# Stability-AI/stable-audio-tools

Measured on AMD Instinct MI355X. Metric: train-step samples/sec (47s@44.1kHz), higher is better.
Workload: dtype f32(bf16x3)

## Files before the change

### include/sat_amd.h

```cpp
#ifndef SAT_AMD_H
#define SAT_AMD_H

#ifdef __cplusplus
extern "C" {
#endif

int sat_abi_version(void);
int sat_is_simulator(void);
const char* sat_last_error(void);


int sat_conv1d(const float* x, const float* w_packed, const float* bias, const float* alpha, const float* beta,
               const float* res, float* y, const float* x2, const float* alpha2, const float* beta2,
               float* part_da, float* part_db, int B, int Cin, int Cout, int Tin, int Tout, int K, int stride,
               int dil, int pad, int tanh_out, void* stream);
int sat_conv1d_partial_rows(int B, int Tout);

int sat_conv1d_bf16x3(const float* x, const short* w_hi, const short* w_lo, const float* bias, const float* snake_a,
                      const float* snake_ib, const float* res, float* y, const float* x2, const float* alpha2,
                      const float* beta2, float* part_da, float* part_db, int B, int Cin, int Cout, int Tin, int Tout,
                      int K, int stride, int dil, int pad, int tanh_out, void* stream);
int sat_conv1d_bf16x3_emit(const float* x, const short* w_hi, const short* w_lo, const float* bias, const float* snake_a,
                      const float* snake_ib, const float* res, float* y, const float* x2, const float* alpha2,
                      const float* beta2, float* part_da, float* part_db, int B, int Cin, int Cout, int Tin, int Tout,
// ... 28 lines not shown
                  void* em_lo, int B, int Cin, int Cout, int frames, int W, int kh, int kw, int dil_t, float slope, const float* lk_src,
                  float lk_slope, void* stream);
int sat_disc_wgrad_nsplit(int B, int M, int Cin, int kh, int frames, int W);
int sat_disc_wgrad(const float* dy, const float* x, float* partial, int B, int M, int Cin, int frames, int W, int kh, int kw, int dil_t,
                   void* stream);

int sat_conv1d_k7_plane_rows(int Tin, int Tout, int pad);
int sat_conv1d_k7_planes(const float* x, const float* snake_a, const float* snake_ib, short* xp_hi, short* xp_lo, int B, int Cin, int Tin,
                         int rows, void* stream);
long long sat_pack_weights_k7q_size(int D0, int D1, int K, int mode);
int sat_pack_weights_k7q(const float* w, short* hi, short* lo, int D0, int D1, int K, int mode, void* stream);
int sat_conv1d_bf16x3_planesq(const short* xp_hi, const short* xp_lo, int rows, const short* w_hi, const short* w_lo, const float* bias,
                             const float* res, float* y, const float* x2, const float* alpha2, const float* beta2, float* part_da,
                             float* part_db, int B, int Cin, int Cout, int Tin, int Tout, int K, int dil, int pad, int tanh_out,
                             int flags, void* stream);
int sat_convtr1d_bf16x3_partial_rows(int B, int Tout, int stride, int pad);
int sat_pack_weights_bf16x3(const float* w, short* hi, short* lo, int D0, int D1, int K, int stride, int mode, void* stream);
long long sat_pack_weights_bf16x3_size(int D0, int D1, int K, int stride, int mode);
int sat_snake_consts(const float* alpha, const float* beta, float* a, float* ib, int C, void* stream);

int sat_convtr1d(const float* x, const float* w_packed, const float* bias, const float* alpha, const float* beta,
                 const float* res, float* y, const float* x2, const float* alpha2, const float* beta2,
                 float* part_da, float* part_db, int B, int Cin, int Cout, int Tin, int Tout, int K, int stride,
                 int pad, int tanh_out, void* stream);
int sat_convtr1d_partial_rows(int B, int Tout, int stride, int pad);

int sat_conv_wgrad(const float* lo, const float* hi, const float* alpha, const float* beta, int snake_on,
                   float* partial, long long so_m, long long so_n, long long so_k, int B, int M, int N, int Tlo,
                   int Thi, int K, int stride, int dil, int pad, void* stream);
int sat_conv_wgrad_nsplit(int B, int M, int N, int Tlo, int K, int stride, int dil);
// ... 162 lines not shown
```

### stable_audio_tools_amd/_lib.py

```python
import ctypes
import os

_P = ctypes.c_void_p
_I = ctypes.c_int
_L = ctypes.c_longlong
_F = ctypes.c_float

SIGNATURES = {
    "sat_abi_version": (_I, []),
    "sat_is_simulator": (_I, []),
    "sat_last_error": (ctypes.c_char_p, []),
    "sat_conv1d": (_I, [_P] * 12 + [_I] * 10 + [_P]),
    "sat_conv1d_partial_rows": (_I, [_I, _I]),
    "sat_conv1d_bf16x3": (_I, [_P] * 13 + [_I] * 10 + [_P]),
    "sat_conv1d_bf16x3_emit": (_I, [_P] * 13 + [_I] * 10 + [_P] * 4 + [_I, _P]),
    "sat_convtr1d_bf16x3": (_I, [_P] * 13 + [_I] * 9 + [_P]),
    "sat_conv1d_bf16x3_partial_rows": (_I, [_I] * 4),
    "sat_rows_pack": (_I, [_P, _P] + [_I] * 10 + [_P]),
    "sat_rows_pack_bwd": (_I, [_P, _P] + [_I] * 10 + [_P]),
    "sat_rows_unpack": (_I, [_P, _P] + [_I] * 6 + [_F, _P]),
    "sat_rows_unpack_bwd": (_I, [_P, _P, _P] + [_I] * 6 + [_F, _P]),
    "sat_disc_geom": (_I, [_I, _I, _P, _P, _P, _P]),
    "sat_disc_planes": (_I, [_P] * 7 + [_I] * 5 + [_F, _P]),
    "sat_disc_l1_blocks": (_I, []),
    "sat_disc_l1_sum": (_I, [_P, _P, _P, _P, _L, _P]),
    "sat_disc_pack_size": (_L, [_I] * 5),
    "sat_disc_pack_weights": (_I, [_P] * 2 + [_I] * 5 + [_P]),
    "sat_disc_conv": (_I, [_P] * 7 + [_I] * 8 + [_F, _P, _F, _P]),
    "sat_disc_wgrad_nsplit": (_I, [_I] * 6),
    "sat_disc_wgrad": (_I, [_P] * 3 + [_I] * 8 + [_P]),
    "sat_conv1d_k7_plane_rows": (_I, [_I] * 3),
    "sat_conv1d_k7_planes": (_I, [_P] * 5 + [_I] * 4 + [_P]),
    "sat_conv1d_bf16x3_planesq": (_I, [_P, _P, _I] + [_P] * 10 + [_I] * 10 + [_P]),
    "sat_pack_weights_k7q": (_I, [_P, _P, _P, _I, _I, _I, _I, _P]),
    "sat_residual_unit_fwd": (_I, [_P, _P, _I] + [_P] * 11 + [_I] * 6 + [_P] * 4 + [_I, _P]),
    "sat_pack_weights_k7q_size": (_L, [_I, _I, _I, _I]),
    "sat_convtr1d_bf16x3_partial_rows": (_I, [_I] * 4),
    "sat_pack_weights_bf16x3": (_I, [_P, _P, _P, _I, _I, _I, _I, _I, _P]),
    "sat_pack_weights_bf16x3_size": (_L, [_I, _I, _I, _I, _I]),
    "sat_snake_consts": (_I, [_P, _P, _P, _P, _I, _P]),
    "sat_conv_wgrad7_bf16x3": (_I, [_P] * 5 + [_L] * 3 + [_I] * 6 + [_P, _P]),
    "sat_conv_wgrad7_bf16x3_nsplit": (_I, [_I] * 4),
    "sat_conv_wgrad7_bf16x3_fuses_rowsum": (_I, [_I] * 4),
    "sat_conv_wgrad_bf16x3": (_I, [_P] * 4 + [_I, _P] + [_L] * 3 + [_I] * 8 + [_P, _P]),
    "sat_conv_wgrad_bf16x3_nsplit": (_I, [_I] * 6),
    "sat_convtr1d": (_I, [_P] * 12 + [_I] * 9 + [_P]),
    "sat_convtr1d_partial_rows": (_I, [_I, _I, _I, _I]),
    "sat_conv_wgrad": (_I, [_P, _P, _P, _P, _I, _P, _L, _L, _L] + [_I] * 9 + [_P]),
    "sat_conv_wgrad_nsplit": (_I, [_I] * 7),
    "sat_reduce_splits": (_I, [_P, _P, _L, _I, _F, _I, _P]),
    "sat_ru_k1_bwd_nsplit": (_I, [_I] * 3),
# ... 101 lines not shown
```

### stable_audio_tools_amd/csrc/conv1d_bf16x3.hip

```cpp
#include "conv_common.h"
#include <type_traits>

#define SAT_K7P_LEAD_ROWS 32
#define SAT_BF_AROWS1 192
#define SAT_BF_AROWSN 136

struct SatConvBfLaunch {
    SatConvParams p;
    const short* w_hi;
    const short* w_lo;
    int cout_pad;
    int cin_v, cout_v;
    int sin_log2;
    int sout_log2;
    int in_shift, out_shift;
    int nq;
    const short* xp_hi = nullptr;
    const short* xp_lo = nullptr;
    int xp_rows = 0, xp_c8 = 0;
    int wq = 0;
    int stagger = 0;
    int persist = 0;
    int dma_in_mfma = 0;
    short* em_hi = nullptr;
    short* em_lo = nullptr;
    const float* em_a = nullptr;
    const float* em_ib = nullptr;
    int em_rows = 0, em_c8 = 0;
    const short* ru_w1_hi = nullptr;
    const short* ru_w1_lo = nullptr;
    const float* ru_bias2 = nullptr;
    const float* ru_a2 = nullptr;
    const float* ru_ib2 = nullptr;
    float* ru_h = nullptr;
};

SAT_DEVICE void sat_split2(float x, short* hi, short* lo) {
    const short h = sat_f32_to_bf16(x);
// ... 672 lines not shown
    if (!em_hi) { sat_set_error("sat_conv1d_bf16x3_emit: planes missing"); return 1; }
    return sat_conv1d_bf16x3_impl("sat_conv1d_bf16x3_emit", x, w_hi, w_lo, bias, snake_a, snake_ib, res, y, x2, alpha2, beta2, part_da, part_db,
                                  B, Cin, Cout, Tin, Tout, K, stride, dil, pad, tanh_out, (short*)em_hi, (short*)em_lo, em_a, em_ib, em_rows, stream);
}

extern "C" int sat_conv1d_k7_plane_rows(int Tin, int Tout, int pad) {
    if (Tin <= 0 || Tout <= 0 || pad < 0 || pad > SAT_K7P_LEAD) return -1;
    const int need = sat_cdiv(Tout, SAT_K7_T) * SAT_K7_T - pad + SAT_K7_AROWS;
    const int body = need > Tin ? need : Tin;
    return SAT_K7P_LEAD + sat_cdiv(body, 64) * 64;
}
extern "C" int sat_conv1d_k7_planes(const float* x, const float* snake_a, const float* snake_ib, short* xp_hi, short* xp_lo, int B,
                                    int Cin, int Tin, int rows, void* stream) {
    if (B <= 0 || Cin <= 0 || Tin <= 0 || rows < SAT_K7P_LEAD + Tin) { sat_set_error("sat_conv1d_k7_planes: bad shape"); return 1; }
    if ((snake_a == nullptr) != (snake_ib == nullptr)) { sat_set_error("sat_conv1d_k7_planes: snake constants must both be given"); return 1; }
    SatK7PlaneParams p{x, snake_a, snake_ib, xp_hi, xp_lo, B, Cin, Tin, rows, sat_cdiv(Cin, 8)};
    SAT_LAUNCH(sat_k7_planes_kernel, dim3(sat_cdiv(rows, 256), p.c8, B), dim3(256), stream, p);
    return sat_check_launch("sat_conv1d_k7_planes");
}
extern "C" int sat_conv1d_bf16x3_planesq(const short* xp_hi, const short* xp_lo, int rows, const short* w_hi, const short* w_lo,
                                         const float* bias, const float* res, float* y, const float* x2, const float* alpha2,
                                         const float* beta2, float* part_da, float* part_db, int B, int Cin, int Cout, int Tin, int Tout,
                                         int K, int dil, int pad, int tanh_out, int flags, void* stream) {
    if (B <= 0 || Cin <= 0 || Cout <= 0 || Tin <= 0 || Tout <= 0) { sat_set_error("sat_conv1d_bf16x3_planesq: empty shape"); return 1; }
    if (K < 5 || K > SAT_K7Q_TAPS || dil < 1 || (K - 1) * dil > 62) {
        sat_set_error("sat_conv1d_bf16x3_planesq: needs stride 1, 5 <= K <= 7, (K-1)*dil <= 62");
        return 1;
    }
    if (rows < sat_conv1d_k7_plane_rows(Tin, Tout, pad)) { sat_set_error("sat_conv1d_bf16x3_planesq: rows must be >= sat_conv1d_k7_plane_rows(Tin, Tout, pad)"); return 1; }
    if (x2 && (!alpha2 || !beta2 || !part_da || !part_db)) { sat_set_error("sat_conv1d_bf16x3_planesq: backward epilogue needs alpha2/beta2/partials"); return 1; }
    SatConvBfLaunch a;
// ... 8 lines not shown
    a.sout_log2 = 0;
    a.in_shift = 0;
    a.out_shift = 0;
    a.nq = Tout;
    a.xp_hi = xp_hi;
    a.xp_lo = xp_lo;
    a.xp_rows = rows;
    a.xp_c8 = sat_cdiv(Cin, 8);
    a.wq = 1;
    a.dma_in_mfma = (flags & 4) ? 1 : 0;
    a.persist = (flags & 1) ? 0 : ((flags & 2) ? 2 : 1);
    SatBfPlan pl{8, 1, K};
    return sat_bf_launch("sat_conv1d_bf16x3_planesq", a, pl, stream);
}

extern "C" int sat_residual_unit_fwd(const short* xp_hi, const short* xp_lo, int rows, const short* w7_hi, const short* w7_lo,
                                     const float* bias1, const float* a2, const float* ib2, const short* w1_hi, const short* w1_lo,
                                     const float* bias2, const float* x, float* h, float* y, int B, int C, int T, int K, int dil, int pad,
                                     void* em_hi, void* em_lo, const float* em_a, const float* em_ib, int em_rows, void* stream) {
    if (B <= 0 || C <= 0 || T <= 0 || C > SAT_K7_CO) { sat_set_error("sat_residual_unit_fwd: needs 1 <= C <= 128"); return 1; }
    if (K < 5 || K > SAT_K7Q_TAPS || dil < 1 || (K - 1) * dil > 62 || 2 * pad != (K - 1) * dil) {
        sat_set_error("sat_residual_unit_fwd: needs 5 <= K <= 7, (K-1)*dil <= 62, 'same' padding");
        return 1;
    }
    if (rows < sat_conv1d_k7_plane_rows(T, T, pad)) { sat_set_error("sat_residual_unit_fwd: rows must be >= sat_conv1d_k7_plane_rows(T, T, pad)"); return 1; }
    if (!xp_hi || !xp_lo || !w7_hi || !w7_lo || !w1_hi || !w1_lo || !a2 || !ib2 || !x || !y) { sat_set_error("sat_residual_unit_fwd: missing operand"); return 1; }
    if ((T & 3) || (((uintptr_t)y | (uintptr_t)x) & 15)) { sat_set_error("sat_residual_unit_fwd: T % 4 == 0 and 16-byte aligned x / y"); return 1; }
    SatConvBfLaunch a;
    a.p = SatConvParams{nullptr, nullptr, bias1, nullptr, nullptr, x, y, nullptr, nullptr, nullptr, nullptr, nullptr,
                        B, C, C, T, T, K, 1, dil, pad, 0};
// ... 57 lines not shown
```

### stable_audio_tools_amd/csrc/conv1d_bf16x3_k7q.h

```cpp
#pragma once

#define SAT_K7Q_TAPS 7
#define SAT_K7Q_WBYTES (2 * SAT_K7Q_TAPS * 2 * 2048)
#define SAT_K7Q_ABYTES (2 * 2 * SAT_K7_AROWS * 16)
#define SAT_K7Q_STAGE (SAT_K7Q_WBYTES + SAT_K7Q_ABYTES)
#define SAT_K7Q_WPIECES (2 * SAT_K7Q_TAPS * 2 * 2)
#define SAT_K7Q_APIECES (2 * 2 * (SAT_K7_AROWS / 64))
#define SAT_K7Q_PIECES (SAT_K7Q_WPIECES + SAT_K7Q_APIECES)

struct SatPackQParams {
    const float* w;
    short* hi;
    short* lo;
    int D0, D1, K, mode, m_v, v_v, out_pad;
    long long total;
};
__global__ void __launch_bounds__(256) sat_pack_k7q_kernel(SatPackQParams p) {
    const long long o = (long long)blockIdx.x * 256 + threadIdx.x;
    if (o >= p.total) return;
    const int e = (int)(o & 7);
    long long q = o >> 3;
    const int m = (int)(q % p.out_pad);
    q /= p.out_pad;
    const int g = (int)(q & 1);
// ... 18 lines not shown
    p->total = (long long)sat_cdiv(p->v_v, 16) * K * 2 * p->out_pad * 8;
    return true;
}
extern "C" long long sat_pack_weights_k7q_size(int D0, int D1, int K, int mode) {
    SatPackQParams p{};
    return sat_pack_q_geometry(D0, D1, K, mode, &p) ? p.total : -1;
}
extern "C" int sat_pack_weights_k7q(const float* w, short* hi, short* lo, int D0, int D1, int K, int mode, void* stream) {
    SatPackQParams p{};
    if (!sat_pack_q_geometry(D0, D1, K, mode, &p)) { sat_set_error("sat_pack_weights_k7q: needs 5 <= K <= 7 (or K == 1: the fused unit's 1x1 conv), mode 0|1"); return 1; }
    p.w = w; p.hi = hi; p.lo = lo;
    SAT_LAUNCH(sat_pack_k7q_kernel, dim3((unsigned)sat_cdivll(p.total, 256)), dim3(256), stream, p);
    return sat_check_launch("sat_pack_weights_k7q");
}

typedef uint32_t u32x2_q __attribute__((ext_vector_type(2)));
template <int VARIANT = 1, bool FUSED = false, bool PERSIST = false>
__global__ void __launch_bounds__(SAT_K7_NT) sat_conv1d_bf16x3_k7q_kernel(SatConvBfLaunch a) {
    static_assert(!(FUSED && PERSIST), "the fused unit is not persistent");
    constexpr bool REORDER = (VARIANT & 1) != 0;
    constexpr bool INMFMA = VARIANT == 3;
    constexpr int CO_T = SAT_K7_CO, T_T = SAT_K7_T, NT = SAT_K7_NT, AROWS = SAT_K7_AROWS;
    constexpr int TW = T_T / 64;
    const SatConvParams& p = a.p;
    constexpr int RED_OFF = 2 * SAT_K7Q_STAGE, EP_OFF = RED_OFF + 2 * TW * CO_T * 4;
    __shared__ __attribute__((aligned(1024))) char lds[EP_OFF + 6 * CO_T * 4];
    float (*red_lds)[TW][CO_T] = reinterpret_cast<float (*)[TW][CO_T]>(lds + RED_OFF);
    float (*ep_lds)[CO_T] = reinterpret_cast<float (*)[CO_T]>(lds + EP_OFF);

    int tid = threadIdx.x;
    int lane = tid & 63;
    int wave = SAT_UNIFORM(tid >> 6);
    int l31 = lane & 31, hi = lane >> 5;
    int wr = wave / TW;
    int co_w = wr * 64, t_w = (wave % TW) * 64;
    const int K = p.K, dil = p.dil;
    const int nchunks = (a.cin_v + 15) / 16;
    const int co_tiles = a.cout_pad / CO_T, t_tiles = (a.nq + T_T - 1) / T_T;
    const int total_tiles = co_tiles * t_tiles * p.B;
    int tile_id = (int)blockIdx.x;
    int co_tile, win;
    sat_xcd_tile(tile_id, co_tiles, t_tiles * p.B, &co_tile, &win);
    int b = win / t_tiles, t_tile = win - b * t_tiles;
    int co0 = co_tile * CO_T, t0 = t_tile * T_T;
    int row_in0 = SAT_K7P_LEAD + t0 - p.pad;
    constexpr int SPAR = PERSIST ? 1 : 0;

    auto load_consts = [&]() {
    if (tid < CO_T) {
        const int m = co0 + tid;
        const bool ok = m < a.cout_v;
        ep_lds[0][tid] = (ok && p.bias) ? p.bias[m] : 0.0f;
// ... 2 lines not shown
        if constexpr (FUSED) {
            ep_lds[1][tid] = ok ? a.ru_a2[m] : 0.0f;
            ep_lds[2][tid] = ok ? a.ru_ib2[m] : 0.0f;
            ep_lds[5][tid] = (ok && a.ru_bias2) ? a.ru_bias2[m] : 0.0f;
        }
        ep_lds[3][tid] = (ok && a.em_a) ? a.em_a[m] : 0.0f;
        ep_lds[4][tid] = (ok && a.em_a) ? a.em_ib[m] : 0.0f;
    }
    };
    load_consts();

    unsigned lane16 = (unsigned)lane * 16u;
    const int w_pl = wave >> 2, w_g = (wave >> 1) & 1, w_half = wave & 1;
    const char* w_src0 = (const char*)(w_pl ? a.w_lo : a.w_hi) + ((size_t)w_g * a.cout_pad + co0 + w_half * 64) * 16;
    const size_t w_tap_stride = (size_t)a.cout_pad * 32;
    const int w_dst0 = w_pl * (SAT_K7Q_TAPS * 4096) + (w_g * 2 + w_half) * 1024;
    auto issue_w = [&](int c, int st, int tap) {
        if (tap < K) sat_glds16(w_src0 + ((size_t)c * K + tap) * w_tap_stride + lane16, lds + st * SAT_K7Q_STAGE + w_dst0 + tap * 4096);
    };
    auto issue_a = [&](int c, int st, int i) {
        const int r = 8 * i + wave;
        if (r < SAT_K7Q_APIECES) {
            const int pl = r / 10, g = (r / 5) & 1, sub = r % 5;
            int c8 = c * 2 + g;
            c8 = c8 < a.xp_c8 ? c8 : a.xp_c8 - 1;
            const char* src = (const char*)(pl ? a.xp_lo : a.xp_hi) + (((size_t)b * a.xp_c8 + c8) * a.xp_rows + row_in0 + sub * 64) * 16;
            sat_glds16(src + lane16, lds + st * SAT_K7Q_STAGE + SAT_K7Q_WBYTES + r * 1024);
        }
    };

    f32x16 acc[2][2];
    auto zero_acc = [&]() {
#pragma unroll
    for (int i = 0; i < 2; ++i)
#pragma unroll
        for (int j = 0; j < 2; ++j)
#pragma unroll
            for (int r = 0; r < 16; ++r) acc[i][j][r] = 0.0f;
    };
    zero_acc();

    struct Frags { bf16x8 wa[2][2], xa[2][2]; };
    Frags fr[4];
    auto load_frags = [&](Frags& f, const char* sb, int tap) {
#pragma unroll
        for (int pl = 0; pl < 2; ++pl) {
            const char* wb = sb + ((pl * SAT_K7Q_TAPS + tap) * 2 + hi) * 2048;
            f.wa[0][pl] = *reinterpret_cast<const bf16x8*>(wb + (co_w + l31) * 16);
            f.wa[1][pl] = *reinterpret_cast<const bf16x8*>(wb + (co_w + 32 + l31) * 16);
            const char* ab = sb + SAT_K7Q_WBYTES + (pl * 2 + hi) * (AROWS * 16);
            f.xa[0][pl] = *reinterpret_cast<const bf16x8*>(ab + (t_w + l31 + tap * dil) * 16);
            f.xa[1][pl] = *reinterpret_cast<const bf16x8*>(ab + (t_w + 32 + l31 + tap * dil) * 16);
        }
    };
    auto mfma_frags = [&](const Frags& f) {
#pragma unroll
        for (int mi = 0; mi < 2; ++mi)
#pragma unroll
            for (int ni = 0; ni < 2; ++ni) acc[mi][ni] = sat_mfma_32x32x16_bf16(f.wa[mi][0], f.xa[ni][0], acc[mi][ni]);
#pragma unroll
        for (int mi = 0; mi < 2; ++mi)
#pragma unroll
            for (int ni = 0; ni < 2; ++ni) acc[mi][ni] = sat_mfma_32x32x16_bf16(f.wa[mi][0], f.xa[ni][1], acc[mi][ni]);
#pragma unroll
        for (int mi = 0; mi < 2; ++mi)
#pragma unroll
            for (int ni = 0; ni < 2; ++ni) acc[mi][ni] = sat_mfma_32x32x16_bf16(f.wa[mi][1], f.xa[ni][0], acc[mi][ni]);
    };

    bool wave_on_co = (co0 + co_w) < a.cout_v;
#if !defined(SAT_HIPEMU)
    if (a.stagger && blockIdx.x < 256) {
        const int steps = (int)((blockIdx.x >> 3) & 7) * a.stagger;
        for (int i = 0; i < steps; ++i) __builtin_amdgcn_s_sleep(127);
    }
#endif
    auto issue_chunk0 = [&]() {
#pragma unroll
        for (int tap = 0; tap < SAT_K7Q_TAPS; ++tap) issue_w(0, SPAR, tap);
        issue_a(0, SPAR, 0); issue_a(0, SPAR, 1); issue_a(0, SPAR, 2);
    };
    issue_chunk0();
  for (;;) {
    SAT_WAIT_VMCNT(0);
    SAT_RAW_BARRIER();
    if (wr == 1) SAT_RAW_BARRIER();

    for (int c = 0; c < nchunks; ++c) {
        const char* sb = lds + ((c + SPAR) & 1) * SAT_K7Q_STAGE;
        const bool more = c + 1 < nchunks;
#pragma unroll
        for (int u = 0; u < 4; ++u) load_frags(fr[u], sb, u);
        if constexpr (INMFMA) {
            SAT_WAIT_VMCNT(0);
        } else if constexpr (REORDER) {
            if (more) {
                issue_a(c + 1, (c + 1 + SPAR) & 1, 0); issue_a(c + 1, (c + 1 + SPAR) & 1, 1); issue_a(c + 1, (c + 1 + SPAR) & 1, 2);
                issue_w(c + 1, (c + 1 + SPAR) & 1, 0); issue_w(c + 1, (c + 1 + SPAR) & 1, 1);
                if (K != SAT_K7Q_TAPS) { SAT_WAIT_VMCNT(0); }
                else if (wave < 4) { SAT_WAIT_VMCNT(5); }
                else { SAT_WAIT_VMCNT(4); }
            } else {
                SAT_WAIT_VMCNT(0);
            }
        } else {
            if (more) {
#pragma unroll
                for (int tap = 0; tap < 5; ++tap) issue_w(c + 1, (c + 1 + SPAR) & 1, tap);
            }
        }
        SAT_WAIT_LGKM0();
        SAT_RAW_BARRIER();
        SAT_SCHED_FENCE();
        SAT_SETPRIO(1);
        if constexpr (INMFMA) {
            const int sn = (c + 1 + SPAR) & 1;
#pragma unroll
            for (int u = 0; u < 4; ++u) {
                if (wave_on_co) mfma_frags(fr[u]);
                SAT_SCHED_FENCE();
                if (more) {
                    if (u == 0) { issue_a(c + 1, sn, 0); issue_a(c + 1, sn, 1); issue_a(c + 1, sn, 2); issue_w(c + 1, sn, 0); }
                    if (u == 1) { issue_w(c + 1, sn, 1); issue_w(c + 1, sn, 2); issue_w(c + 1, sn, 3); }
                }
                SAT_SCHED_FENCE();
            }
        } else
        if (wave_on_co) {
#pragma unroll
            for (int u = 0; u < 4; ++u) mfma_frags(fr[u]);
        }
        SAT_SETPRIO(0);
        SAT_SCHED_FENCE();
        SAT_RAW_BARRIER();
#pragma unroll
        for (int u = 0; u < 3; ++u)
            if (4 + u < K) load_frags(fr[u], sb, 4 + u);
        if constexpr (INMFMA) {
            SAT_WAIT_VMCNT(0);
        } else if constexpr (REORDER) {
            if (more) {
#pragma unroll
                for (int tap = 2; tap < SAT_K7Q_TAPS; ++tap) issue_w(c + 1, (c + 1 + SPAR) & 1, tap);
                if (K == SAT_K7Q_TAPS) { SAT_WAIT_VMCNT(3); } else { SAT_WAIT_VMCNT(0); }
            }
        } else if (more) {
            issue_w(c + 1, (c + 1 + SPAR) & 1, 5); issue_w(c + 1, (c + 1 + SPAR) & 1, 6);
            issue_a(c + 1, (c + 1 + SPAR) & 1, 0); issue_a(c + 1, (c + 1 + SPAR) & 1, 1); issue_a(c + 1, (c + 1 + SPAR) & 1, 2);
            SAT_WAIT_VMCNT(0);
        }
        SAT_WAIT_LGKM0();
        SAT_RAW_BARRIER();
        SAT_SCHED_FENCE();
        SAT_SETPRIO(1);
        if constexpr (INMFMA) {
            const int sn = (c + 1 + SPAR) & 1;
#pragma unroll
            for (int u = 0; u < 3; ++u) {
                if (wave_on_co && 4 + u < K) mfma_frags(fr[u]);
                SAT_SCHED_FENCE();
                if (more) issue_w(c + 1, sn, 4 + u);
                SAT_SCHED_FENCE();
            }
        } else
        if (wave_on_co) {
#pragma unroll
            for (int u = 0; u < 3; ++u)
                if (4 + u < K) mfma_frags(fr[u]);
        }
        SAT_SETPRIO(0);
        SAT_SCHED_FENCE();
        SAT_RAW_BARRIER();
    }
    if (wr == 0) SAT_RAW_BARRIER();
    __syncthreads();
    const int e_b = b, e_t_tile = t_tile, e_co0 = co0, e_t0 = t0;
// ... 275 lines not shown
        hi = lane >> 5;
        lane16 = (unsigned)lane * 16u;
        wr = wave / TW;
        co_w = wr * 64;
        t_w = (wave % TW) * 64;
    }
  }
}

static void sat_bf_launch_k7q(SatConvBfLaunch& a, void* stream) {
    const long long total = (long long)(a.cout_pad / SAT_K7_CO) * sat_cdiv(a.nq, SAT_K7_T) * a.p.B;
    a.stagger = 1;
    if (total < 1024) a.stagger = 0;
    if (a.ru_w1_hi) { SAT_LAUNCH((sat_conv1d_bf16x3_k7q_kernel<1, true>), dim3((unsigned)total), dim3(SAT_K7_NT), stream, a); return; }
    const int cus = sat_cu_count();
    if (a.persist == 2 && total >= 2) {
        a.stagger = 0;
        if (a.dma_in_mfma) { SAT_LAUNCH((sat_conv1d_bf16x3_k7q_kernel<3, false, true>), dim3((unsigned)sat_cdivll(total, 3)), dim3(SAT_K7_NT), stream, a); }
        else { SAT_LAUNCH((sat_conv1d_bf16x3_k7q_kernel<1, false, true>), dim3((unsigned)sat_cdivll(total, 3)), dim3(SAT_K7_NT), stream, a); }
        return;
    }
    if (a.persist && total >= 2 * cus) {
        if (a.dma_in_mfma) { SAT_LAUNCH((sat_conv1d_bf16x3_k7q_kernel<3, false, true>), dim3((unsigned)cus), dim3(SAT_K7_NT), stream, a); }
        else { SAT_LAUNCH((sat_conv1d_bf16x3_k7q_kernel<1, false, true>), dim3((unsigned)cus), dim3(SAT_K7_NT), stream, a); }
        return;
    }
    if (a.dma_in_mfma) { SAT_LAUNCH((sat_conv1d_bf16x3_k7q_kernel<3>), dim3((unsigned)total), dim3(SAT_K7_NT), stream, a); }
    else { SAT_LAUNCH((sat_conv1d_bf16x3_k7q_kernel<1>), dim3((unsigned)total), dim3(SAT_K7_NT), stream, a); }
}
```

### stable_audio_tools_amd/csrc/conv1d_planes.h

```cpp
#pragma once

#define SAT_K7P_LEAD 32
static_assert(SAT_K7P_LEAD == SAT_K7P_LEAD_ROWS, "plane emission (conv1d_bf16x3.hip) writes row 32 + t");

struct SatK7PlaneParams {
    const float* x;
    const float* a;
    const float* ib;
    short* hi;
    short* lo;
    int B, Cin, Tin, rows, c8;
};

__global__ void __launch_bounds__(256) sat_k7_planes_kernel(SatK7PlaneParams p) {
    const int row = blockIdx.x * 256 + threadIdx.x;
    const int chunk = blockIdx.y, b = blockIdx.z;
    if (row >= p.rows) return;
    const int t = row - SAT_K7P_LEAD;
    const bool t_ok = (unsigned)t < (unsigned)p.Tin;
    uint32_t h[4], l[4];
#pragma unroll
    for (int j = 0; j < 4; ++j) {
        float v[2];
#pragma unroll
        for (int e = 0; e < 2; ++e) {
            const int ch = chunk * 8 + 2 * j + e;
            const int chc = ch < p.Cin ? ch : p.Cin - 1;
            const bool ok = t_ok && ch < p.Cin;
            float o = ok ? p.x[((size_t)b * p.Cin + chc) * p.Tin + t] : 0.0f;
            if (p.a) o = sat_snake(o, p.a[chc], p.ib[chc]);
            v[e] = o;
        }
        sat_split2_pk(v[0], v[1], &h[j], &l[j]);
    }
    const size_t o = (((size_t)b * p.c8 + chunk) * p.rows + row) * 8;
    *reinterpret_cast<u32x4*>(p.hi + o) = u32x4{h[0], h[1], h[2], h[3]};
    *reinterpret_cast<u32x4*>(p.lo + o) = u32x4{l[0], l[1], l[2], l[3]};
}
```

### stable_audio_tools_amd/functional.py

```python
import torch

from . import ops as _ops_mod
from .ops import PACK_CONV_DGRAD, PACK_CONV_FWD, PACK_POLYPHASE


def _ops(ops):
    return ops if ops is not None else _ops_mod.get_ops()


class SumAllFn(torch.autograd.Function):

    @staticmethod
    def forward(ctx, x, ops=None):
        ctx.in_shape, ctx.in_dtype = x.shape, x.dtype
        return _ops(ops).sum_all(x.detach())

    @staticmethod
    def backward(ctx, g):
        return g.to(ctx.in_dtype).expand(ctx.in_shape), None


def sum_all(x, ops=None):
    return SumAllFn.apply(x, ops)

# ... 76 lines not shown
    w, norm = ops.wn_fold(v, gf)
    return w, (v, gf, norm)


def _wn_backward(ops, slabs, saved, g_shape, bias_partial=None):
    v, gf, norm = saved
    out = ops.wn_grad_splits(slabs, v, gf, norm, bias_partial=bias_partial)
    return (out[0], out[1].view(g_shape)) + tuple(out[2:])


def _conv_fwd(ops, x, w, stride, dil, pad, bias=None, snake=None, res=None, tanh_out=False, dsnake=None, tout=None, cache=None, emit=None):
    cout, cin, k = w.shape
    if (res is None and ops.edge_ok(cin, cout, k, stride, dil, pad) and (tout is None or tout == x.shape[2])
            and (snake is None or cout <= 2) and (dsnake is None or cin <= 2) and (emit is None or cin <= 2)):
        return ops.edge_conv(x, w, pad, bias=bias, snake=snake, tanh_out=tanh_out, dsnake=dsnake, emit=emit)
    if ops.bf16x3_ok(k, stride, dil):
        q = ops.k7q_applicable(cin, k, stride, dil, pad, cout)
        planes = _cached(cache, "pack_fwd_q" if q else "pack_fwd", (w,), lambda: ops.pack_bf16x3(w, stride=stride, q=q))
        sconsts = _cached(cache, "snake", snake, lambda: ops.snake_consts(snake[0], snake[1])) if snake is not None else None
        return ops.conv1d_bf16x3(x, planes, cout, k, stride, dil, pad, tout=tout, bias=bias,
                                 snake=snake, res=res, tanh_out=tanh_out, dsnake=dsnake, sconsts=sconsts, emit=emit)
    return ops.conv1d(x, _cached(cache, "pack_fwd32", (w,), lambda: ops.pack(w, PACK_CONV_FWD)), cout, k, stride, dil, pad, tout=tout,
                      bias=bias, snake=snake, res=res, tanh_out=tanh_out, dsnake=dsnake)


def _convtr_fwd(ops, x, w, stride, pad, bias=None, snake=None, cache=None):
    cin, cout, k = w.shape
    if ops.bf16x3_ok(k, stride, 1, transposed=True):
        planes = _cached(cache, "pack_tr", (w,), lambda: ops.pack_bf16x3(w, mode=2, stride=stride))
        sconsts = _cached(cache, "snake", snake, lambda: ops.snake_consts(snake[0], snake[1])) if snake is not None else None
# ... 200 lines not shown
```

### stable_audio_tools_amd/ops.py

```python
import ctypes

import torch

from . import _caches, _lib

PACK_CONV_FWD = 0
PACK_CONV_DGRAD = 1
PACK_POLYPHASE = 2


def _ptr(t):
    if t is None:
        return None
    return ctypes.c_void_p(t.data_ptr())


def _keep_zeros(shape, dtype, device):
    with torch.inference_mode(False):
        return torch.zeros(shape, dtype=dtype, device=device)


def _keep_empty(shape, dtype, device):
    with torch.inference_mode(False):
        return torch.empty(shape, dtype=dtype, device=device)
# ... 188 lines not shown
        if transposed or stride > 1:
            return k == 2 * stride and stride & (stride - 1) == 0 and dil == 1
        return k == 1 or (2 <= k <= 4 and dil == 1) or (5 <= k <= 8 and (k - 1) * dil <= 62)

    k7q = True
    k7q_persist = True
    k7q_dma_in_mfma = True
    k7q_min_cin = 64
    k7q_min_cout = 128
    k7q_wide_cin = 512

    def k7q_applicable(self, cin, k, stride, dil, pad, cout=None):
        return (self.k7q and self.use_bf16x3 and stride == 1 and 5 <= k <= 7 and 0 <= pad <= 32
                and (k - 1) * dil <= 62 and cin >= self.k7q_min_cin
                and (cout is None or cout >= self.k7q_min_cout or cin >= self.k7q_wide_cin))

    def pack_bf16x3(self, w, mode=0, stride=1, q=False):
        self._f32(w)
        d0, d1, k = w.shape
        if q:
            n = self.lib.sat_pack_weights_k7q_size(d0, d1, k, mode)
            if n <= 0 or stride != 1:
                raise RuntimeError("sat_pack_weights_k7q: unsupported shape")
            hi = torch.empty(n, dtype=torch.int16, device=w.device)
            lo = torch.empty(n, dtype=torch.int16, device=w.device)
            self._chk(self.lib.sat_pack_weights_k7q(_ptr(w), _ptr(hi), _ptr(lo), d0, d1, k, mode, self._stream(w)))
            return hi, lo, "q"
        n = self.lib.sat_pack_weights_bf16x3_size(d0, d1, k, stride, mode)
        if n <= 0:
            raise RuntimeError("sat_pack_weights_bf16x3: unsupported shape")
# ... 1104 lines not shown
```

Before: 7.783.

## Route strided K=2S conv1d through space-to-depth planes on the k7q MFMA kernel

Adds a space-to-depth path for strided downsampling convolutions with K=2*stride. The input is split into S phase planes, so the strided conv becomes a stride-1, two-tap conv over Cin*S channels and runs on the existing pipelined k7q bf16x3 MFMA kernel, with a matching weight packer. It applies when Cin*S >= 4096 and Cout >= 128, and is meant to replace the slower generic strided bf16x3 kernel for the encoder downsampling layers. The cost is an extra plane-materialisation pass and workspace memory per call.

```diff
diff --git a/include/sat_amd.h b/include/sat_amd.h
--- a/include/sat_amd.h
+++ b/include/sat_amd.h
@@ -66,6 +66,15 @@
                              const float* res, float* y, const float* x2, const float* alpha2, const float* beta2, float* part_da,
                              float* part_db, int B, int Cin, int Cout, int Tin, int Tout, int K, int dil, int pad, int tanh_out,
                              int flags, void* stream);
+int sat_conv1d_s2d_plane_rows(int Tin, int Tout, int S);
+int sat_conv1d_s2d_planes(const float* x, const float* snake_a, const float* snake_ib, short* xp_hi, short* xp_lo, int B, int Cin,
+                          int Tin, int S, int rows, void* stream);
+long long sat_pack_weights_s2d_size(int D0, int D1, int S, int pad);
+int sat_pack_weights_s2d(const float* w, short* hi, short* lo, int D0, int D1, int S, int pad, void* stream);
+int sat_conv1d_bf16x3_s2d(const short* xp_hi, const short* xp_lo, int rows, const short* w_hi, const short* w_lo, const float* bias,
+                          const float* res, float* y, const float* x2, const float* alpha2, const float* beta2, float* part_da,
+                          float* part_db, int B, int Cin, int Cout, int Tin, int Tout, int S, int pad, int tanh_out, void* em_hi,
+                          void* em_lo, const float* em_a, const float* em_ib, int em_rows, int flags, void* stream);
 int sat_convtr1d_bf16x3_partial_rows(int B, int Tout, int stride, int pad);
 int sat_pack_weights_bf16x3(const float* w, short* hi, short* lo, int D0, int D1, int K, int stride, int mode, void* stream);
 long long sat_pack_weights_bf16x3_size(int D0, int D1, int K, int stride, int mode);
diff --git a/stable_audio_tools_amd/_lib.py b/stable_audio_tools_amd/_lib.py
--- a/stable_audio_tools_amd/_lib.py
+++ b/stable_audio_tools_amd/_lib.py
@@ -35,6 +35,11 @@
     "sat_pack_weights_k7q": (_I, [_P, _P, _P, _I, _I, _I, _I, _P]),
     "sat_residual_unit_fwd": (_I, [_P, _P, _I] + [_P] * 11 + [_I] * 6 + [_P] * 4 + [_I, _P]),
     "sat_pack_weights_k7q_size": (_L, [_I, _I, _I, _I]),
+    "sat_conv1d_s2d_plane_rows": (_I, [_I] * 3),
+    "sat_conv1d_s2d_planes": (_I, [_P] * 5 + [_I] * 5 + [_P]),
+    "sat_pack_weights_s2d": (_I, [_P] * 3 + [_I] * 4 + [_P]),
+    "sat_pack_weights_s2d_size": (_L, [_I] * 4),
+    "sat_conv1d_bf16x3_s2d": (_I, [_P, _P, _I] + [_P] * 10 + [_I] * 8 + [_P] * 4 + [_I, _I, _P]),
     "sat_convtr1d_bf16x3_partial_rows": (_I, [_I] * 4),
     "sat_pack_weights_bf16x3": (_I, [_P, _P, _P, _I, _I, _I, _I, _I, _P]),
     "sat_pack_weights_bf16x3_size": (_L, [_I, _I, _I, _I, _I]),
diff --git a/stable_audio_tools_amd/csrc/conv1d_bf16x3.hip b/stable_audio_tools_amd/csrc/conv1d_bf16x3.hip
--- a/stable_audio_tools_amd/csrc/conv1d_bf16x3.hip
+++ b/stable_audio_tools_amd/csrc/conv1d_bf16x3.hip
@@ -22,6 +22,8 @@
     int stagger = 0;
     int persist = 0;
     int dma_in_mfma = 0;
+    int s2d_stride = 0;
+    int s2d_pad = 0, s2d_c8 = 0;
     short* em_hi = nullptr;
     short* em_lo = nullptr;
     const float* em_a = nullptr;
@@ -724,7 +726,7 @@
                                     int Cin, int Tin, int rows, void* stream) {
     if (B <= 0 || Cin <= 0 || Tin <= 0 || rows < SAT_K7P_LEAD + Tin) { sat_set_error("sat_conv1d_k7_planes: bad shape"); return 1; }
     if ((snake_a == nullptr) != (snake_ib == nullptr)) { sat_set_error("sat_conv1d_k7_planes: snake constants must both be given"); return 1; }
-    SatK7PlaneParams p{x, snake_a, snake_ib, xp_hi, xp_lo, B, Cin, Tin, rows, sat_cdiv(Cin, 8)};
+    SatK7PlaneParams p{x, snake_a, snake_ib, xp_hi, xp_lo, B, Cin, Tin, rows, sat_cdiv(Cin, 8), 1};
     SAT_LAUNCH(sat_k7_planes_kernel, dim3(sat_cdiv(rows, 256), p.c8, B), dim3(256), stream, p);
     return sat_check_launch("sat_conv1d_k7_planes");
 }
@@ -763,6 +765,57 @@
     return sat_bf_launch("sat_conv1d_bf16x3_planesq", a, pl, stream);
 }
 
+extern "C" int sat_conv1d_s2d_plane_rows(int Tin, int Tout, int S) {
+    if (Tin <= 0 || Tout <= 0 || S < 2) return -1;
+    return sat_conv1d_k7_plane_rows(sat_cdiv(Tin, S), Tout, 0);
+}
+extern "C" int sat_conv1d_s2d_planes(const float* x, const float* snake_a, const float* snake_ib, short* xp_hi, short* xp_lo, int B,
+                                     int Cin, int Tin, int S, int rows, void* stream) {
+    if (B <= 0 || Cin <= 0 || (Cin & 7) || Tin <= 0 || S < 2 || rows < SAT_K7P_LEAD + sat_cdiv(Tin, S)) { sat_set_error("sat_conv1d_s2d_planes: bad shape"); return 1; }
+    if ((snake_a == nullptr) != (snake_ib == nullptr)) { sat_set_error("sat_conv1d_s2d_planes: snake constants must both be given"); return 1; }
+    SatK7PlaneParams p{x, snake_a, snake_ib, xp_hi, xp_lo, B, Cin, Tin, rows, Cin / 8, S};
+    SAT_LAUNCH(sat_k7_planes_kernel, dim3(sat_cdiv(rows, 256), S * p.c8, B), dim3(256), stream, p);
+    return sat_check_launch("sat_conv1d_s2d_planes");
+}
+extern "C" int sat_conv1d_bf16x3_s2d(const short* xp_hi, const short* xp_lo, int rows, const short* w_hi, const short* w_lo,
+                                     const float* bias, const float* res, float* y, const float* x2, const float* alpha2,
+                                     const float* beta2, float* part_da, float* part_db, int B, int Cin, int Cout, int Tin, int Tout,
+                                     int S, int pad, int tanh_out, void* em_hi, void* em_lo, const float* em_a, const float* em_ib,
+                                     int em_rows, int flags, void* stream) {
+    if (B <= 0 || Cin <= 0 || Cout <= 0 || Tin <= 0 || Tout <= 0) { sat_set_error("sat_conv1d_bf16x3_s2d: empty shape"); return 1; }
+    if ((Cin & 7) || S < 2 || S > 64 || pad < 1 || pad > S) { sat_set_error("sat_conv1d_bf16x3_s2d: needs Cin % 8 == 0, 2 <= S <= 64, 1 <= pad <= S"); return 1; }
+    if (rows < sat_conv1d_s2d_plane_rows(Tin, Tout, S)) { sat_set_error("sat_conv1d_bf16x3_s2d: rows must be >= sat_conv1d_s2d_plane_rows(Tin, Tout, S)"); return 1; }
+    if (x2 && (!alpha2 || !beta2 || !part_da || !part_db)) { sat_set_error("sat_conv1d_bf16x3_s2d: backward epilogue needs alpha2/beta2/partials"); return 1; }
+    SatConvBfLaunch a;
+    a.p = SatConvParams{nullptr, nullptr, bias, nullptr, nullptr, res, y, x2, alpha2, beta2, part_da, part_db,
+                        B, Cin, Cout, Tin, Tout, 4, 1, 1, 1, tanh_out};
+    a.w_hi = w_hi;
+    a.w_lo = w_lo;
+    a.cout_v = Cout;
+    a.cout_pad = sat_cdiv(Cout, SAT_CO_T) * SAT_CO_T;
+    a.cin_v = Cin * S;
+    a.sin_log2 = 0; a.sout_log2 = 0; a.in_shift = 0; a.out_shift = 0;
+    a.nq = Tout;
+    a.xp_hi = xp_hi;
+    a.xp_lo = xp_lo;
+    a.xp_rows = rows;
+    a.xp_c8 = S * (Cin / 8);
+    a.wq = 1;
+    a.dma_in_mfma = 1;
+    a.persist = (flags & 1) ? 0 : ((flags & 2) ? 2 : 1);
+    a.s2d_stride = S; a.s2d_pad = pad; a.s2d_c8 = Cin / 8;
+    if (em_hi) {
+        if (!em_lo || (em_a == nullptr) != (em_ib == nullptr) || em_rows < SAT_K7P_LEAD_ROWS + Tout || (Tout & 3) ||
+            (((uintptr_t)em_hi | (uintptr_t)em_lo | (uintptr_t)y | (uintptr_t)x2 | (uintptr_t)res) & 15)) {
+            sat_set_error("sat_conv1d_bf16x3_s2d: emission needs Tout % 4 == 0, 16-byte aligned tensors, rows >= 32 + Tout");
+            return 1;
+        }
+        a.em_hi = (short*)em_hi; a.em_lo = (short*)em_lo; a.em_a = em_a; a.em_ib = em_ib; a.em_rows = em_rows; a.em_c8 = sat_cdiv(Cout, 8);
+    }
+    SatBfPlan pl{8, 1, 4};
+    return sat_bf_launch("sat_conv1d_bf16x3_s2d", a, pl, stream);
+}
+
 extern "C" int sat_residual_unit_fwd(const short* xp_hi, const short* xp_lo, int rows, const short* w7_hi, const short* w7_lo,
                                      const float* bias1, const float* a2, const float* ib2, const short* w1_hi, const short* w1_lo,
                                      const float* bias2, const float* x, float* h, float* y, int B, int C, int T, int K, int dil, int pad,
diff --git a/stable_audio_tools_amd/csrc/conv1d_bf16x3_k7q.h b/stable_audio_tools_amd/csrc/conv1d_bf16x3_k7q.h
--- a/stable_audio_tools_amd/csrc/conv1d_bf16x3_k7q.h
+++ b/stable_audio_tools_amd/csrc/conv1d_bf16x3_k7q.h
@@ -56,10 +56,66 @@
     return sat_check_launch("sat_pack_weights_k7q");
 }
 
+struct SatPackS2dParams {
+    const float* w;
+    short* hi;
+    short* lo;
+    int D0, D1, S, pad, v_v, out_pad;
+    long long total;
+};
+__global__ void __launch_bounds__(256) sat_pack_s2d_kernel(SatPackS2dParams p) {
+    const long long o = (long long)blockIdx.x * 256 + threadIdx.x;
+    if (o >= p.total) return;
+    const int e = (int)(o & 7);
+    long long q = o >> 3;
+    const int m = (int)(q % p.out_pad);
+    q /= p.out_pad;
+    const int g = (int)(q & 1);
+    q >>= 1;
+    const int j = (int)(q & 3), chunk = (int)(q >> 2);
+    const int v = ((chunk * 2 + (j >> 1)) * 2 + g) * 8 + e;
+    float val = 0.0f;
+    if (m < p.D0 && v < p.v_v) {
+        const int r = v / p.D1, ci = v - r * p.D1;
+        const int k = p.S * ((r + p.pad < p.S ? 0 : -1) + (j & 1)) + r + p.pad;
+        val = p.w[((size_t)m * p.D1 + ci) * (2 * p.S) + k];
+    }
+    short h, l;
+    sat_split2(val, &h, &l);
+    p.hi[o] = h;
+    p.lo[o] = l;
+}
+static bool sat_pack_s2d_geometry(int D0, int D1, int S, int pad, SatPackS2dParams* p) {
+    if (D0 <= 0 || D1 <= 0 || (D1 & 7) || S < 2 || S > 64 || pad < 1 || pad > S) return false;
+    p->D0 = D0; p->D1 = D1; p->S = S; p->pad = pad;
+    p->v_v = D1 * S;
+    p->out_pad = sat_cdiv(D0, SAT_K7_CO) * SAT_K7_CO;
+    p->total = (long long)sat_cdiv(p->v_v, 32) * 4 * 2 * p->out_pad * 8;
+    return true;
+}
+extern "C" long long sat_pack_weights_s2d_size(int D0, int D1, int S, int pad) {
+    SatPackS2dParams p{};
+    return sat_pack_s2d_geometry(D0, D1, S, pad, &p) ? p.total : -1;
+}
+extern "C" int sat_pack_weights_s2d(const float* w, short* hi, short* lo, int D0, int D1, int S, int pad, void* stream) {
+    SatPackS2dParams p{};
+    if (!sat_pack_s2d_geometry(D0, D1, S, pad, &p)) { sat_set_error("sat_pack_weights_s2d: needs K = 2S, 2 <= S <= 64, 1 <= pad <= S, D1 % 8 == 0"); return 1; }
+    p.w = w; p.hi = hi; p.lo = lo;
+    SAT_LAUNCH(sat_pack_s2d_kernel, dim3((unsigned)sat_cdivll(p.total, 256)), dim3(256), stream, p);
+    return sat_check_launch("sat_pack_weights_s2d");
+}
+
 typedef uint32_t u32x2_q __attribute__((ext_vector_type(2)));
-template <int VARIANT = 1, bool FUSED = false, bool PERSIST = false>
+template <int VARIANT = 1, bool FUSED = false, bool PERSIST = false, bool S2D = false>
 __global__ void __launch_bounds__(SAT_K7_NT) sat_conv1d_bf16x3_k7q_kernel(SatConvBfLaunch a) {
     static_assert(!(FUSED && PERSIST), "the fused unit is not persistent");
+    static_assert(!S2D || (VARIANT == 3 && !FUSED), "the space-to-depth chunks run the VARIANT 3 K loop only");
+    constexpr int NTAPS = S2D ? 4 : SAT_K7Q_TAPS;
+    constexpr int TAPS0 = S2D ? 2 : 4;
+    constexpr int A_OFF = S2D ? 2 * NTAPS * 4096 : SAT_K7Q_WBYTES;
+    constexpr int APIECES = S2D ? 2 * SAT_K7Q_APIECES : SAT_K7Q_APIECES;
+    constexpr int AISSUE = (APIECES + 7) / 8;
+    static_assert(A_OFF + APIECES * 1024 <= SAT_K7Q_STAGE, "stage overflow");
     constexpr bool REORDER = (VARIANT & 1) != 0;
     constexpr bool INMFMA = VARIANT == 3;
     constexpr int CO_T = SAT_K7_CO, T_T = SAT_K7_T, NT = SAT_K7_NT, AROWS = SAT_K7_AROWS;
@@ -77,7 +133,7 @@
     int wr = wave / TW;
     int co_w = wr * 64, t_w = (wave % TW) * 64;
     const int K = p.K, dil = p.dil;
-    const int nchunks = (a.cin_v + 15) / 16;
+    const int nchunks = S2D ? (a.cin_v + 31) / 32 : (a.cin_v + 15) / 16;
     const int co_tiles = a.cout_pad / CO_T, t_tiles = (a.nq + T_T - 1) / T_T;
     const int total_tiles = co_tiles * t_tiles * p.B;
     int tile_id = (int)blockIdx.x;
@@ -110,18 +166,21 @@
     const int w_pl = wave >> 2, w_g = (wave >> 1) & 1, w_half = wave & 1;
     const char* w_src0 = (const char*)(w_pl ? a.w_lo : a.w_hi) + ((size_t)w_g * a.cout_pad + co0 + w_half * 64) * 16;
     const size_t w_tap_stride = (size_t)a.cout_pad * 32;
-    const int w_dst0 = w_pl * (SAT_K7Q_TAPS * 4096) + (w_g * 2 + w_half) * 1024;
+    const int w_dst0 = w_pl * (NTAPS * 4096) + (w_g * 2 + w_half) * 1024;
     auto issue_w = [&](int c, int st, int tap) {
         if (tap < K) sat_glds16(w_src0 + ((size_t)c * K + tap) * w_tap_stride + lane16, lds + st * SAT_K7Q_STAGE + w_dst0 + tap * 4096);
     };
     auto issue_a = [&](int c, int st, int i) {
         const int r = 8 * i + wave;
-        if (r < SAT_K7Q_APIECES) {
-            const int pl = r / 10, g = (r / 5) & 1, sub = r % 5;
-            int c8 = c * 2 + g;
+        if (r < APIECES) {
+            const int s = S2D ? r / SAT_K7Q_APIECES : 0, rr = S2D ? r % SAT_K7Q_APIECES : r;
+            const int pl = rr / 10, g = (rr / 5) & 1, sub = rr % 5;
+            int c8 = (S2D ? c * 4 + s * 2 : c * 2) + g;
             c8 = c8 < a.xp_c8 ? c8 : a.xp_c8 - 1;
-            const char* src = (const char*)(pl ? a.xp_lo : a.xp_hi) + (((size_t)b * a.xp_c8 + c8) * a.xp_rows + row_in0 + sub * 64) * 16;
-            sat_glds16(src + lane16, lds + st * SAT_K7Q_STAGE + SAT_K7Q_WBYTES + r * 1024);
+            int row = row_in0 + sub * 64;
+            if constexpr (S2D) row += sat_s2d_shift(c8, a.s2d_c8, a.s2d_stride, a.s2d_pad);
+            const char* src = (const char*)(pl ? a.xp_lo : a.xp_hi) + (((size_t)b * a.xp_c8 + c8) * a.xp_rows + row) * 16;
+            sat_glds16(src + lane16, lds + st * SAT_K7Q_STAGE + A_OFF + r * 1024);
         }
     };
 
@@ -141,12 +200,13 @@
     auto load_frags = [&](Frags& f, const char* sb, int tap) {
 #pragma unroll
         for (int pl = 0; pl < 2; ++pl) {
-            const char* wb = sb + ((pl * SAT_K7Q_TAPS + tap) * 2 + hi) * 2048;
+            const char* wb = sb + ((pl * NTAPS + tap) * 2 + hi) * 2048;
             f.wa[0][pl] = *reinterpret_cast<const bf16x8*>(wb + (co_w + l31) * 16);
             f.wa[1][pl] = *reinterpret_cast<const bf16x8*>(wb + (co_w + 32 + l31) * 16);
-            const char* ab = sb + SAT_K7Q_WBYTES + (pl * 2 + hi) * (AROWS * 16);
-            f.xa[0][pl] = *reinterpret_cast<const bf16x8*>(ab + (t_w + l31 + tap * dil) * 16);
-            f.xa[1][pl] = *reinterpret_cast<const bf16x8*>(ab + (t_w + 32 + l31 + tap * dil) * 16);
+            const int sub = S2D ? tap >> 1 : 0, roff = S2D ? (tap & 1) : tap * dil;
+            const char* ab = sb + A_OFF + ((sub * 2 + pl) * 2 + hi) * (AROWS * 16);
+            f.xa[0][pl] = *reinterpret_cast<const bf16x8*>(ab + (t_w + l31 + roff) * 16);
+            f.xa[1][pl] = *reinterpret_cast<const bf16x8*>(ab + (t_w + 32 + l31 + roff) * 16);
         }
     };
     auto mfma_frags = [&](const Frags& f) {
@@ -173,8 +233,9 @@
 #endif
     auto issue_chunk0 = [&]() {
 #pragma unroll
-        for (int tap = 0; tap < SAT_K7Q_TAPS; ++tap) issue_w(0, SPAR, tap);
-        issue_a(0, SPAR, 0); issue_a(0, SPAR, 1); issue_a(0, SPAR, 2);
+        for (int tap = 0; tap < NTAPS; ++tap) issue_w(0, SPAR, tap);
+#pragma unroll
+        for (int i = 0; i < AISSUE; ++i) issue_a(0, SPAR, i);
     };
     issue_chunk0();
   for (;;) {
@@ -186,7 +247,7 @@
         const char* sb = lds + ((c + SPAR) & 1) * SAT_K7Q_STAGE;
         const bool more = c + 1 < nchunks;
 #pragma unroll
-        for (int u = 0; u < 4; ++u) load_frags(fr[u], sb, u);
+        for (int u = 0; u < TAPS0; ++u) load_frags(fr[u], sb, u);
         if constexpr (INMFMA) {
             SAT_WAIT_VMCNT(0);
         } else if constexpr (REORDER) {
@@ -212,12 +273,17 @@
         if constexpr (INMFMA) {
             const int sn = (c + 1 + SPAR) & 1;
 #pragma unroll
-            for (int u = 0; u < 4; ++u) {
+            for (int u = 0; u < TAPS0; ++u) {
                 if (wave_on_co) mfma_frags(fr[u]);
                 SAT_SCHED_FENCE();
                 if (more) {
-                    if (u == 0) { issue_a(c + 1, sn, 0); issue_a(c + 1, sn, 1); issue_a(c + 1, sn, 2); issue_w(c + 1, sn, 0); }
-                    if (u == 1) { issue_w(c + 1, sn, 1); issue_w(c + 1, sn, 2); issue_w(c + 1, sn, 3); }
+                    if constexpr (S2D) {
+                        if (u == 0) { issue_a(c + 1, sn, 0); issue_a(c + 1, sn, 1); issue_a(c + 1, sn, 2); }
+                        if (u == 1) { issue_a(c + 1, sn, 3); issue_a(c + 1, sn, 4); issue_w(c + 1, sn, 0); issue_w(c + 1, sn, 1); }
+                    } else {
+                        if (u == 0) { issue_a(c + 1, sn, 0); issue_a(c + 1, sn, 1); issue_a(c + 1, sn, 2); issue_w(c + 1, sn, 0); }
+                        if (u == 1) { issue_w(c + 1, sn, 1); issue_w(c + 1, sn, 2); issue_w(c + 1, sn, 3); }
+                    }
                 }
                 SAT_SCHED_FENCE();
             }
@@ -231,7 +297,7 @@
         SAT_RAW_BARRIER();
 #pragma unroll
         for (int u = 0; u < 3; ++u)
-            if (4 + u < K) load_frags(fr[u], sb, 4 + u);
+            if (TAPS0 + u < K) load_frags(fr[u], sb, TAPS0 + u);
         if constexpr (INMFMA) {
             SAT_WAIT_VMCNT(0);
         } else if constexpr (REORDER) {
@@ -253,9 +319,9 @@
             const int sn = (c + 1 + SPAR) & 1;
 #pragma unroll
             for (int u = 0; u < 3; ++u) {
-                if (wave_on_co && 4 + u < K) mfma_frags(fr[u]);
+                if (wave_on_co && TAPS0 + u < K) mfma_frags(fr[u]);
                 SAT_SCHED_FENCE();
-                if (more) issue_w(c + 1, sn, 4 + u);
+                if (more) issue_w(c + 1, sn, TAPS0 + u);
                 SAT_SCHED_FENCE();
             }
         } else
@@ -561,6 +627,13 @@
     if (total < 1024) a.stagger = 0;
     if (a.ru_w1_hi) { SAT_LAUNCH((sat_conv1d_bf16x3_k7q_kernel<1, true>), dim3((unsigned)total), dim3(SAT_K7_NT), stream, a); return; }
     const int cus = sat_cu_count();
+    if (a.s2d_stride) {
+        a.stagger = 0;
+        if (a.persist == 2 && total >= 2) { SAT_LAUNCH((sat_conv1d_bf16x3_k7q_kernel<3, false, true, true>), dim3((unsigned)sat_cdivll(total, 3)), dim3(SAT_K7_NT), stream, a); }
+        else if (a.persist == 1 && total >= 2 * cus) { SAT_LAUNCH((sat_conv1d_bf16x3_k7q_kernel<3, false, true, true>), dim3((unsigned)cus), dim3(SAT_K7_NT), stream, a); }
+        else { SAT_LAUNCH((sat_conv1d_bf16x3_k7q_kernel<3, false, false, true>), dim3((unsigned)total), dim3(SAT_K7_NT), stream, a); }
+        return;
+    }
     if (a.persist == 2 && total >= 2) {
         a.stagger = 0;
         if (a.dma_in_mfma) { SAT_LAUNCH((sat_conv1d_bf16x3_k7q_kernel<3, false, true>), dim3((unsigned)sat_cdivll(total, 3)), dim3(SAT_K7_NT), stream, a); }
diff --git a/stable_audio_tools_amd/csrc/conv1d_planes.h b/stable_audio_tools_amd/csrc/conv1d_planes.h
--- a/stable_audio_tools_amd/csrc/conv1d_planes.h
+++ b/stable_audio_tools_amd/csrc/conv1d_planes.h
@@ -9,14 +9,20 @@
     const float* ib;
     short* hi;
     short* lo;
-    int B, Cin, Tin, rows, c8;
+    int B, Cin, Tin, rows, c8, S;
 };
+
+SAT_DEVICE int sat_s2d_shift(int c8, int cin8, int S, int pad) {
+    const int r = c8 / cin8;
+    return r + pad < S ? 1 : 0;
+}
 
 __global__ void __launch_bounds__(256) sat_k7_planes_kernel(SatK7PlaneParams p) {
     const int row = blockIdx.x * 256 + threadIdx.x;
-    const int chunk = blockIdx.y, b = blockIdx.z;
+    const int pchunk = blockIdx.y, b = blockIdx.z;
     if (row >= p.rows) return;
-    const int t = row - SAT_K7P_LEAD;
+    const int phase = pchunk / p.c8, chunk = pchunk - phase * p.c8;
+    const int t = (row - SAT_K7P_LEAD) * p.S + phase;
     const bool t_ok = (unsigned)t < (unsigned)p.Tin;
     uint32_t h[4], l[4];
 #pragma unroll
@@ -33,7 +39,7 @@
         }
         sat_split2_pk(v[0], v[1], &h[j], &l[j]);
     }
-    const size_t o = (((size_t)b * p.c8 + chunk) * p.rows + row) * 8;
+    const size_t o = (((size_t)b * p.S * p.c8 + pchunk) * p.rows + row) * 8;
     *reinterpret_cast<u32x4*>(p.hi + o) = u32x4{h[0], h[1], h[2], h[3]};
     *reinterpret_cast<u32x4*>(p.lo + o) = u32x4{l[0], l[1], l[2], l[3]};
 }
diff --git a/stable_audio_tools_amd/functional.py b/stable_audio_tools_amd/functional.py
--- a/stable_audio_tools_amd/functional.py
+++ b/stable_audio_tools_amd/functional.py
@@ -114,6 +114,11 @@
     if (res is None and ops.edge_ok(cin, cout, k, stride, dil, pad) and (tout is None or tout == x.shape[2])
             and (snake is None or cout <= 2) and (dsnake is None or cin <= 2) and (emit is None or cin <= 2)):
         return ops.edge_conv(x, w, pad, bias=bias, snake=snake, tanh_out=tanh_out, dsnake=dsnake, emit=emit)
+    if ops.bf16x3_ok(k, stride, dil) and ops.strided_planes_ok(cin, cout, k, stride, pad):
+        planes = _cached(cache, "pack_s2d", (w,), lambda: ops.pack_s2d(w, stride, pad))
+        sconsts = _cached(cache, "snake", snake, lambda: ops.snake_consts(snake[0], snake[1])) if snake is not None else None
+        return ops.conv1d_s2d(x, planes, cout, stride, pad, tout=tout, bias=bias, snake=snake, res=res, tanh_out=tanh_out,
+                              dsnake=dsnake, sconsts=sconsts, emit=emit)
     if ops.bf16x3_ok(k, stride, dil):
         q = ops.k7q_applicable(cin, k, stride, dil, pad, cout)
         planes = _cached(cache, "pack_fwd_q" if q else "pack_fwd", (w,), lambda: ops.pack_bf16x3(w, stride=stride, q=q))
diff --git a/stable_audio_tools_amd/ops.py b/stable_audio_tools_amd/ops.py
--- a/stable_audio_tools_amd/ops.py
+++ b/stable_audio_tools_amd/ops.py
@@ -226,6 +226,69 @@
         return (self.k7q and self.use_bf16x3 and stride == 1 and 5 <= k <= 7 and 0 <= pad <= 32
                 and (k - 1) * dil <= 62 and cin >= self.k7q_min_cin
                 and (cout is None or cout >= self.k7q_min_cout or cin >= self.k7q_wide_cin))
+
+    strided_planes = True
+    strided_planes_min_cin_v = 4096
+
+    def strided_planes_ok(self, cin, cout, k, stride, pad):
+        return (self.strided_planes and self.use_bf16x3 and stride > 1 and k == 2 * stride and stride & (stride - 1) == 0
+                and 1 <= pad <= stride and cin % 8 == 0 and cout >= self.k7q_min_cout and cin * stride >= self.strided_planes_min_cin_v)
+
+    def pack_s2d(self, w, stride, pad):
+        self._f32(w)
+        d0, d1, _ = w.shape
+        n = self.lib.sat_pack_weights_s2d_size(d0, d1, stride, pad)
+        if n <= 0:
+            raise RuntimeError("sat_pack_weights_s2d: unsupported shape")
+        hi = torch.empty(n, dtype=torch.int16, device=w.device)
+        lo = torch.empty(n, dtype=torch.int16, device=w.device)
+        self._chk(self.lib.sat_pack_weights_s2d(_ptr(w), _ptr(hi), _ptr(lo), d0, d1, stride, pad, self._stream(w)))
+        return hi, lo, "s2d"
+
+    def conv1d_s2d(self, x, w_planes, cout, stride, pad, tout=None, bias=None, snake=None, res=None, tanh_out=False, dsnake=None,
+                   sconsts=None, emit=None):
+        b, cin, tin = x.shape
+        k = 2 * stride
+        if tout is None:
+            tout = (tin + 2 * pad - k) // stride + 1
+        self._f32(x, bias, res)
+        sa = sib = None
+        if snake is not None:
+            sa, sib = sconsts if sconsts is not None else self.snake_consts(snake[0], snake[1])
+        st = self._stream(x)
+        rows = self.lib.sat_conv1d_s2d_plane_rows(tin, tout, stride)
+        need = 2 * b * (stride * cin // 8) * rows * 8
+        wkey = ("k7p", x.device, st.value if st is not None else 0)
+        ws = self.__dict__.setdefault("_planes", {}).get(wkey)
+        if ws is None or ws.numel() < need:
+            ws = _keep_empty(need, torch.int16, x.device)
+            self._planes[wkey] = ws
+        hi, lo = ws[:need // 2], ws[need // 2:need]
+        self._chk(self.lib.sat_conv1d_s2d_planes(_ptr(x), _ptr(sa), _ptr(sib), _ptr(hi), _ptr(lo), b, cin, tin, stride, rows, st))
+        y = torch.empty(b, cout, tout, dtype=torch.float32, device=x.device)
+        x2 = a2 = b2 = pda = pdb = None
+        if dsnake is not None:
+            x2, a2, b2 = dsnake
+            self._f32(x2, a2, b2)
+            prows = b * ((tout + 255) // 256)
+            pda, pdb = torch.empty(2, cout, prows, dtype=torch.float32, device=x.device).unbind(0)
+        ehi = elo = ea = eib = None
+        erows = 0
+        esnake = None
+        if emit is not None:
+            esnake = emit.get("snake")
+            if esnake is not None:
+                ea, eib = self.snake_consts(esnake[0], esnake[1])
+            ehi, elo, erows = self._emit_planes(b, cout, tout, x.device, st)
+        self._chk(self.lib.sat_conv1d_bf16x3_s2d(_ptr(hi), _ptr(lo), rows, _ptr(w_planes[0]), _ptr(w_planes[1]), _ptr(bias), _ptr(res),
+                                                 _ptr(y), _ptr(x2), _ptr(a2), _ptr(b2), _ptr(pda), _ptr(pdb), b, cin, cout, tin, tout,
+                                                 stride, pad, int(tanh_out), _ptr(ehi), _ptr(elo), _ptr(ea), _ptr(eib), erows,
+                                                 {True: 0, False: 1, "force": 2}[self.k7q_persist], st))
+        if emit is not None:
+            self._note_emitted(y, esnake, ehi, elo, erows)
+        if dsnake is not None:
+            return (y, *self._sum_pair(pda, pdb))
+        return y
 
     def pack_bf16x3(self, w, mode=0, stride=1, q=False):
         self._f32(w)
```

Measured after the change: 7.802 (median of 6 runs). About the same (+0.2%).
